# emilemathieu/RiemannHamiltonianMonteCarlo

Measured on AMD Instinct MI355X. Metric: leapfrog-steps/sec (whole node), higher is better.
Workload: dtype f64 (the two O(M D^2) contractions as exact int8-sliced integer GEMMs)

## Files before the change

### riemannhamiltonianmontecarlo_amd/csrc/metric_i8.hip.h

```cpp
#pragma once
#include <hip/hip_runtime.h>
#include <stdint.h>
#include <utility>
#include "plan.h"

typedef int i4v __attribute__((ext_vector_type(4)));
typedef int i16v __attribute__((ext_vector_type(16)));

#define I8_ROWB 32
__device__ __forceinline__ int i8_lds_off(int row, int half) { return row * I8_ROWB + ((half ^ ((row >> 3) & 1)) << 4); }

#ifndef I8_GC
#define I8_GC 4
#define I8_GP 8
#endif
#ifndef I8_DSPREAD
#define I8_DSPREAD 1
#endif
__device__ __forceinline__ bool i8_tile_of_block(int b, int nCB, int nPB, int& cb, int& pb) {
  if (nCB < 8) {
    if (b >= nCB * nPB) return false;
    cb = b % nCB;
    pb = b / nCB;
    return true;
// ... 41 lines not shown
}
#ifndef I8_ASMFRAG
#define I8_ASMFRAG 1
#endif

#ifndef I8_ABLATE
#define I8_ABLATE 0
#endif
template <int S, class F>
__device__ __forceinline__ double i8_combine(F&& acc_of) {
  double val = 0.0;
#pragma unroll
  for (int g = S - 1; g >= 0; --g) val = val * 0.00390625 + (double)acc_of(g);
  return val;
}

#ifndef I8_NBUF4
#define I8_NBUF4 1
#endif
template <int S, int WN, int TN>
constexpr int i8_nbuf() {
  constexpr int ROWS = I8_BM + 32 * TN * WN, NT = 128 * WN, NU = (2 * ROWS + NT - 1) / NT;
  return (I8_NBUF4 && S <= 4 && 2 * ROWS == NU * NT && 4 * S * ROWS * 32 <= 140 * 1024) ? 4 : 3;
}

template <int S, int WN, int TN, int PIN, bool RAW = false, class Epilogue>
__device__ __forceinline__ void gemm_i8_tile(const int8_t* __restrict__ Vs, const int8_t* __restrict__ Zs, int nCp, int NPp, int nks_total, int nks,
                                             int cb, int pb, int rows_real, int cols_real, Epilogue&& epi) {
  constexpr int BM = I8_BM, BN = 32 * TN * WN, ROWS = BM + BN, NT = 128 * WN;
  constexpr int STAGE = S * ROWS * I8_ROWB;
  constexpr int NU = (2 * ROWS + NT - 1) / NT;
  static_assert((2 * ROWS) % 64 == 0, "whole waves of 16-byte units");
  extern __shared__ __attribute__((aligned(16))) unsigned char lds[];
  const int t = threadIdx.x, lane = t & 63, wave = t >> 6;
  const int wm = wave & 1, wn = wave >> 1;
  const size_t strideV = (size_t)nks_total * nCp * 32, strideZ = (size_t)nks_total * NPp * 32;
  const int8_t* gbase[NU];
  size_t gstep[NU], gslice[NU];
  unsigned goff[NU];
  int lbase[NU];
  bool on[NU];
  int n_on = 0;
#pragma unroll
  for (int k = 0; k < NU; ++k) {
    const int u = t + k * NT;
    on[k] = (u & ~63) < 2 * ROWS;
// ... 120 lines not shown
        for (int a = 0; a < 2; ++a) fa[(i + 1) & 1][a] = *(const i4v*)(bc + (i + 1) * ROWS * I8_ROWB + fragA + a * 32 * I8_ROWB);
      }
      if (spread && (ALLON || ks + PD < nks)) gl1(kpre, wr, i);
      if (PIN) __builtin_amdgcn_sched_barrier(0);
#pragma unroll
      for (int j = S - 1 - i; j >= 0; --j) {
#pragma unroll
        for (int a = 0; a < 2; ++a)
#pragma unroll
          for (int b = 0; b < TN; ++b)
            acc[i + j][a][b] = __builtin_amdgcn_mfma_i32_32x32x32_i8(fa[i & 1][a], fb[j][b], acc[i + j][a][b], 0, 0, 0);
        if (PIN && i == 0) __builtin_amdgcn_sched_barrier(0);
      }
      if (PIN) __builtin_amdgcn_sched_barrier(0);
    }
    }
    }
    if constexpr (NBUF == 3) { if (ALLON || ks + 2 < nks) retire_older(); else wait_vmcnt<0>(); }
    else wait_vmcnt<(PD - 1) * S * NU>();
    if (!(I8_ABLATE & 4)) __builtin_amdgcn_s_barrier();
    cur = nxt;
  }
  if (ALLON) wait_vmcnt<0>();
#pragma unroll
  for (int a = 0; a < 2; ++a)
#pragma unroll
    for (int b = 0; b < TN; ++b)
#pragma unroll
      for (int r = 0; r < 16; ++r) {
        const int row = cb * BM + wm * 64 + a * 32 + (r & 3) + 8 * (r >> 2) + 4 * (lane >> 5);
        const int col = pb * BN + wn * 32 * TN + b * 32 + (lane & 31);
        if constexpr (RAW) {
#pragma unroll
          for (int g = 0; g < S; ++g) epi(row, col, g, acc[g][a][b][r]);
        } else {
          epi(row, col, i8_combine<S>([&](int g) { return acc[g][a][b][r]; }));
        }
      }
}

template <int S, int WN, int TN>
constexpr int i8_lds_bytes() { return i8_nbuf<S, WN, TN>() * S * (I8_BM + 32 * TN * WN) * I8_ROWB; }

template <int S, int WN, int TN, int PIN>
__global__ __launch_bounds__(128 * WN) __attribute__((amdgpu_waves_per_eu(WN >= 2 ? WN / 2 : 1, WN >= 4 ? WN / 2 : 2))) void k_gemm_i8_probe(const int8_t* __restrict__ Vs, const int8_t* __restrict__ Zs, int nCp, int NPp, int nks,
                                                            int nC, int NP, double* __restrict__ C) {
  int cb, pb;
  if (!i8_tile_of_block(blockIdx.x, nCp / I8_BM, NPp / (32 * TN * WN), cb, pb)) return;
  gemm_i8_tile<S, WN, TN, PIN>(Vs, Zs, nCp, NPp, nks, nks, cb, pb, nC - cb * I8_BM, NP - pb * 32 * TN * WN,
                          [&](int row, int col, double val) {
#ifdef I8_PROBE_NOSTORE
                            if (val == 1.2345e300)
#endif
                            C[(size_t)row * NPp + col] = val; });
}

template <int S>
__device__ __forceinline__ void split_digits(long long N, int (&d)[S]) {
#pragma unroll
  for (int k = 0; k < S; ++k) {
    const int b = (int)(signed char)(N & 0xFF);
    d[k] = b;
    N = (N - b) >> 8;
  }
}

struct I8Pairs {
  const short* pa;
  const short* pb;
  const double* scale;
  int NP, NPp;
  const int* cexp;
};

__global__ __launch_bounds__(256) void k_zmax(const double* __restrict__ Xt, int M, int Mp, I8Pairs pr, int* __restrict__ ze,
                                              double* __restrict__ scale) {
  __shared__ double red[256];
// ... 150 lines not shown

struct I8Delta {
  const unsigned long long* dsel;
  const int* rebase;
  double cscale;
  int need_lo, need_hi;
  const double* Gbase;
  unsigned long long* count = nullptr;
  __device__ __forceinline__ bool skip() const;
};
__device__ __forceinline__ int i8_delta_slices(unsigned long long bits) {
  const double mx = __longlong_as_double((long long)bits);
  if (mx <= 0.49 * 4294967296.0) return 4;
  if (mx <= 0.49 * 1099511627776.0) return 5;
  return 6;
}

__device__ __forceinline__ bool I8Delta::skip() const {
  if (!dsel) return false;
  const int need = i8_delta_slices(*dsel);
  return need < need_lo || need > need_hi;
}

template <int S, int WN, int TN>
__device__ __forceinline__ void assemble_i8_body(const int8_t* __restrict__ Vs, const int8_t* __restrict__ Zs, int nCp, int nks_total,
                                                 int ks0, int nk, int accumulate, const I8Pairs& pr, int n_chains, const int* __restrict__ phase,
                                                 const int* __restrict__ vbad, int DP, double inv_alpha, double* __restrict__ Gq,
                                                 size_t plane_stride, const int* __restrict__ vexp, int npb, const I8Delta& dl) {
  int cb, pb;
  if (!i8_tile_of_block(blockIdx.x, nCp / I8_BM, npb, cb, pb)) return;
  const int per = (nk + (int)gridDim.y - 1) / (int)gridDim.y;
  const int kb = ks0 + (int)blockIdx.y * per, kn = min(per, ks0 + nk - kb);
  double* __restrict__ Gout = Gq + (size_t)blockIdx.y * plane_stride;
  const bool first = blockIdx.y == 0;
  constexpr int BN = 32 * TN * WN;
  __shared__ double s_cmul[I8_BM];
  __shared__ double s_pscale[BN];
  __shared__ int s_coff[I8_BM];
  __shared__ int s_poff[BN];
  for (int i = threadIdx.x; i < I8_BM + BN; i += 128 * WN) {
    if (i < I8_BM) {
      const int c = cb * I8_BM + i;
      const bool ok = c < n_chains && phase[min(c, n_chains - 1)] == 1;
      s_coff[i] = ok ? ((dl.rebase && dl.rebase[c]) ? 3 : 1) : 0;
      s_cmul[i] = ok ? (vbad[c] ? __builtin_nan("") : ldexp(dl.cscale, -vexp[c])) : 0.0;
    } else {
      const int j = i - I8_BM, p = pb * BN + j;
      const bool ok = p < pr.NP;
      const int a = ok ? pr.pa[p] : 0, b = ok ? pr.pb[p] : 0;
      s_poff[j] = ok ? a * DP + b : -1;
      s_pscale[j] = ok ? (a == b ? -pr.scale[p] : pr.scale[p]) : 0.0;
    }
  }
  __syncthreads();
  gemm_i8_tile<S, WN, TN, (WN == 4)>(Vs + (size_t)kb * nCp * 32, Zs + (size_t)kb * pr.NPp * 32, nCp, pr.NPp, nks_total, kn, cb, pb,
                                     n_chains - cb * I8_BM, pr.NP - pb * 32 * TN * WN, [&](int c, int p, double val) {
    const int ci = c - cb * I8_BM, pj = p - pb * BN;
    const int off = s_poff[pj];
    const double ps = s_pscale[pj];
    const bool ok = s_coff[ci] != 0 && off >= 0;
    double* gp = Gout + (size_t)min(c, n_chains - 1) * DP * DP + max(off, 0);
    double g = (val * fabs(ps)) * s_cmul[ci];
    if (accumulate & 1) g += *gp;
    else if ((accumulate & 2) && s_coff[ci] != 3) g += dl.Gbase ? dl.Gbase[(size_t)min(c, n_chains - 1) * DP * DP + max(off, 0)] : *gp;
    else if (ps < 0.0 && first) g += inv_alpha;
    if (ok) *gp = g;
  });
}
template <int S, int WN, int TN>
__global__ __launch_bounds__(128 * WN) __attribute__((amdgpu_waves_per_eu(WN / 2, WN / 2))) void k_assemble_i8(const int8_t* __restrict__ Vs, const int8_t* __restrict__ Zs, int nCp, int nks_total,
                                                          int ks0, int nk, int accumulate, I8Pairs pr, int n_chains, const int* __restrict__ phase,
                                                          const int* __restrict__ vbad, int DP, double inv_alpha, double* __restrict__ Gq,
                                                          size_t plane_stride, const int* __restrict__ vexp, int npb, I8Delta dl) {
  if (dl.skip()) return;
  assemble_i8_body<S, WN, TN>(Vs, Zs, nCp, nks_total, ks0, nk, accumulate, pr, n_chains, phase, vbad, DP, inv_alpha, Gq, plane_stride, vexp, npb, dl);
}
__device__ __forceinline__ int i8_delta_pick(const I8Delta& dl, int seff) {
  const int need = i8_delta_slices(*dl.dsel);
  return seff == 6 ? need : (need == 6 ? 5 : 4);
}
__device__ __forceinline__ void i8_delta_count(const I8Delta& dl, int seff, int Sp) {
  if (dl.count && blockIdx.x == 0 && blockIdx.y == 0 && threadIdx.x == 0) atomicAdd(dl.count + 3 * (6 - seff) + (Sp - 4), 1ull);
}
template <int WN, int TN>
__global__ __launch_bounds__(128 * WN) __attribute__((amdgpu_waves_per_eu(WN / 2, WN / 2))) void k_assemble_i8_sel(const int8_t* __restrict__ Vs, size_t vplane, int seff, const int8_t* __restrict__ Zs, int nCp, int nks_total,
                                                          int ks0, int nk, int accumulate, I8Pairs pr, int n_chains, const int* __restrict__ phase,
                                                          const int* __restrict__ vbad, int DP, double inv_alpha, double* __restrict__ Gq,
                                                          size_t plane_stride, const int* __restrict__ vexp, int npb, I8Delta dl) {
  const int Sp = i8_delta_pick(dl, seff);
  i8_delta_count(dl, seff, Sp);
  dl.cscale = __builtin_ldexp(1.0, -8 * (seff - Sp));
  Vs += (size_t)(seff - Sp) * vplane;
  if (Sp == 6) assemble_i8_body<6, WN, TN>(Vs, Zs, nCp, nks_total, ks0, nk, accumulate, pr, n_chains, phase, vbad, DP, inv_alpha, Gq, plane_stride, vexp, npb, dl);
  else if (Sp == 5) assemble_i8_body<5, WN, TN>(Vs, Zs, nCp, nks_total, ks0, nk, accumulate, pr, n_chains, phase, vbad, DP, inv_alpha, Gq, plane_stride, vexp, npb, dl);
  else assemble_i8_body<4, WN, TN>(Vs, Zs, nCp, nks_total, ks0, nk, accumulate, pr, n_chains, phase, vbad, DP, inv_alpha, Gq, plane_stride, vexp, npb, dl);
}

template <int S>
__device__ __forceinline__ void assemble_i8_tail_body(
    const int8_t* __restrict__ Vs, const int8_t* __restrict__ Zs, int nCp, int NPp, int NP, int nks_total, int ks0, int nk, int n_chains, int pb32_0,
    int ntail, int* __restrict__ Tq) {
  const int nCB = nCp / I8_BM;
  const int cb = blockIdx.x % nCB, tb = blockIdx.x / nCB;
  const int per = (nk + (int)gridDim.y - 1) / (int)gridDim.y;
  const int kb = ks0 + (int)blockIdx.y * per, kn = min(per, ks0 + nk - kb);
  int* __restrict__ T = Tq + (size_t)blockIdx.y * S * nCp * 32 * ntail;
  const int pb32 = pb32_0 + tb;
  if (kn <= 0) {
    for (int i = threadIdx.x; i < S * I8_BM * 32; i += 128) {
      const int g = i / (I8_BM * 32), r = i % (I8_BM * 32);
      T[((size_t)g * nCp + cb * I8_BM + (r >> 5)) * 32 * ntail + tb * 32 + (r & 31)] = 0;
    }
    return;
  }
  gemm_i8_tile<S, 1, 1, 0, true>(Vs + (size_t)kb * nCp * 32, Zs + (size_t)kb * NPp * 32, nCp, NPp, nks_total, kn, cb, pb32, n_chains - cb * I8_BM,
                                 NP - pb32 * 32, [&](int c, int p, int g, int a) {
    T[((size_t)g * nCp + c) * 32 * ntail + (p - pb32_0 * 32)] = a;
  });
// ... 160 lines not shown
#pragma unroll
    for (int s = 0; s < S; ++s) w[s] = 0;
#pragma unroll
    for (int k = 0; k < 4; ++k) {
      int d[S];
      split_digits<S>((long long)rint(ldexp(ok ? q[k] : 0.0, shf)), d);
#pragma unroll
      for (int s = 0; s < S; ++s) w[s] |= (d[S - 1 - s] & 0xFF) << (8 * k);
    }
    const int kp = q4 >> 3, k4 = q4 & 7;
#pragma unroll
    for (int s = 0; s < S; ++s) *(int*)(Qs + (((size_t)s * nkp + kp) * nCp + c) * 32 + 4 * k4) = w[s];
  };
#pragma unroll
  for (int i = 0; i < QMAX; ++i)
    if (t + 256 * i < nq) put(t + 256 * i, qv[i]);
  for (int q4 = t + 256 * QMAX; q4 < nq; q4 += 256) {
    double mag;
    const double q[4] = {entry(4 * q4, mag), entry(4 * q4 + 1, mag), entry(4 * q4 + 2, mag), entry(4 * q4 + 3, mag)};
    put(q4, q);
  }
}

template <int S, int WN, int TN>
__global__ __launch_bounds__(128 * WN) __attribute__((amdgpu_waves_per_eu(WN / 2, WN / 2))) void k_leverage_i8(
    const int8_t* __restrict__ Qs, const int8_t* __restrict__ Zt, int nCp, int NRp, int nkp_total, int kp0, int nk, int accumulate, int mulc,
    int n_chains, int Mp, const int* __restrict__ phase, const double* __restrict__ qscale, const double* __restrict__ zscale,
    const double* __restrict__ crow, double* __restrict__ R, size_t plane_stride) {
  int cb, rb;
  if (!i8_tile_of_block(blockIdx.x, nCp / I8_BM, NRp / (32 * TN * WN), cb, rb)) return;
  const int per = (nk + (int)gridDim.y - 1) / (int)gridDim.y;
  const int kb = kp0 + (int)blockIdx.y * per, kn = min(per, kp0 + nk - kb);
  double* __restrict__ Rout = R + (size_t)blockIdx.y * plane_stride;
  constexpr int BN = 32 * TN * WN;
  __shared__ double s_q[I8_BM], s_z[BN];
  __shared__ int s_ok[I8_BM];
  for (int i = threadIdx.x; i < I8_BM + BN; i += 128 * WN) {
    if (i < I8_BM) {
      const int c = cb * I8_BM + i;
      const bool ok = c < n_chains && phase[min(c, n_chains - 1)] == 1;
      s_ok[i] = ok ? 1 : 0;
      s_q[i] = ok ? qscale[c] : 0.0;
    } else {
      const int n = rb * BN + (i - I8_BM);
      s_z[i - I8_BM] = n < NRp ? zscale[n] : 0.0;
    }
  }
  __syncthreads();
  gemm_i8_tile<S, WN, TN, (WN == 4)>(Qs + (size_t)kb * nCp * 32, Zt + (size_t)kb * NRp * 32, nCp, NRp, nkp_total, kn, cb, rb,
                                     n_chains - cb * I8_BM, Mp - rb * 32 * TN * WN, [&](int c, int n, double val) {
    const int ci = c - cb * I8_BM;
    const bool ok = s_ok[ci] != 0 && n < Mp;
    const size_t o = (size_t)min(c, n_chains - 1) * Mp + min(n, Mp - 1);
    double r = val * s_q[ci] * s_z[n - rb * BN];
    if (mulc) r *= crow[o];
    if (accumulate) r += Rout[o];
    if (ok) Rout[o] = r;
  });
}
```

### riemannhamiltonianmontecarlo_amd/csrc/plan.h

```cpp
#pragma once
#include "../../include/rmhmc.h"

#include <stddef.h>
#include <stdint.h>
#include <string.h>

#include <algorithm>

#define RM_LD 66

#define FS_D 8
#define FS_WAVES 4
#define FS_PT 104

#define MS_MAXMP 2048
#define MS_GLD 34

template <int NB>
constexpr int ms_lds_doubles(int Mp) {
  return 64 * RM_LD + 32 * MS_GLD + 4 * (16 * NB) * (16 * NB) + 2 * Mp + 12 * 32 + 4 * 40;
}

#define I8_BM 128
constexpr int i8_tile_wn(int S) { return S <= 6 ? 4 : 2; }
constexpr int i8_tile_tn(int) { return 1; }

#define AMH_MAX_ONCHIP_ROWS (256 * 48)

struct Options {
  int64_t graph = 1, sorted = 1, inflight = 32, cdyn = 1, crestore = 1, i8_force_rebase = 0;
  int64_t ccache = 1, medium = 1, fused = 1, hmc_traj_maxn = -1, fsplit = 0, nsplit_max = 64, nsplit_waves = -1, i8_tail = -1,
          i8_delta = 1, i8_delta_inner = 1;
};
struct OptionDesc { const char* key; int64_t Options::*slot; bool create_only; int64_t lo, hi; };
inline const OptionDesc kOptions[] = {
    {"graph", &Options::graph, false, 0, 1},
    {"sorted", &Options::sorted, false, 0, 1},
    {"inflight", &Options::inflight, false, 0, 1 << 20},
    {"cdyn", &Options::cdyn, false, 0, 1},
    {"crestore", &Options::crestore, false, 0, 1},
    {"i8_force_rebase", &Options::i8_force_rebase, false, 0, 1},
    {"ccache", &Options::ccache, true, 0, 1},
    {"medium", &Options::medium, true, 0, 1},
    {"fused", &Options::fused, true, 0, 1},
    {"hmc_traj_maxn", &Options::hmc_traj_maxn, true, -1, (int64_t)1 << 40},
    {"fsplit", &Options::fsplit, true, 0, 64},
    {"nsplit_max", &Options::nsplit_max, true, 1, 1 << 20},
    {"nsplit_waves", &Options::nsplit_waves, true, -1, 1 << 20},
    {"i8_tail", &Options::i8_tail, true, -1, 1},
    {"i8_delta", &Options::i8_delta, true, 0, 1},
    {"i8_delta_inner", &Options::i8_delta_inner, true, 0, 1},
};
inline const OptionDesc* find_option(const char* key) {
  if (!key) return nullptr;
  for (const OptionDesc& d : kOptions)
    if (!strcmp(d.key, key)) return &d;
  return nullptr;
}
enum OptionError { OPT_OK, OPT_UNKNOWN, OPT_CREATE_ONLY, OPT_RANGE };
inline OptionError check_option(const OptionDesc* d, int64_t value, bool at_create) {
  if (!d) return OPT_UNKNOWN;
  if (d->create_only && !at_create) return OPT_CREATE_ONLY;
  if (value < d->lo || value > d->hi) return OPT_RANGE;
  return OPT_OK;
}

struct PlanCheck { int code; const char* msg; };
inline PlanCheck plan_check(int64_t M, int32_t D, int64_t n_chains, int32_t dtype, uint32_t flags) {
  auto no = [](int code, const char* m) { return PlanCheck{code, m}; };
  if (M <= 0 || D <= 0 || n_chains <= 0) return no(RMHMC_ERR_INVALID, "rmhmc_create: bad shape");
  if (dtype != RMHMC_F64) return no(RMHMC_ERR_UNSUPPORTED, "rmhmc_create: only float64 is built (the reference is float64)");
  if (D > 256) return no(RMHMC_ERR_UNSUPPORTED, "rmhmc_create: D > 256 is not supported (64 < D <= 256 uses the blocked large-D path)");
  if (flags & RMHMC_FLAG_ORACLE_LITERAL) return no(RMHMC_ERR_UNSUPPORTED, "rmhmc_create: the literal variant exists only in the CPU oracle");
  if (M > (int64_t)1 << 30 || n_chains > (int64_t)1 << 30) return no(RMHMC_ERR_UNSUPPORTED, "rmhmc_create: M or n_chains too large");
// ... 138 lines not shown
```

### riemannhamiltonianmontecarlo_amd/csrc/rmhmc_hip.hip

```cpp
#include "../../include/rmhmc.h"
#include "../../include/rmhmc_amh.h"
#include "../../include/rmhmc_iwls.h"
#include "../../include/rmhmc_gibbs.h"
#include "plan.h"
#include "kernels.hip.h"
#include "fused_small.hip.h"
#include "large_d.hip.h"
#include "metric_i8.hip.h"
#include "medium_step.hip.h"
#include "amh.hip.h"
#include "iwls.hip.h"
#include "gibbs.hip.h"

#include <algorithm>
#include <chrono>
#include <cmath>
#include <cstdio>
#include <cstdlib>
#include <cstring>
#include <map>
#include <string>
#include <vector>

namespace {
// ... 202 lines not shown
  });
}

template <int S, int WN, int TN>
void launch_assemble_i8_t(rmhmc_ctx* ctx, Group& g, const double* v, hipStream_t st, int part, bool delta = false, int seff = 6, int need_lo = 0,
                          int need_hi = 0) {
  const size_t vplane = (size_t)ctx->i8_nks * g.nCp * 32;
  const int8_t* const Vs = g.Vs + (delta ? (size_t)(seff - S) * vplane : 0);
  const I8Delta dl{delta ? g.dmax : nullptr, delta ? g.rebase : nullptr, delta ? std::ldexp(1.0, -8 * (seff - S)) : 1.0, need_lo, need_hi,
                   (delta && ctx->big) ? g.Gbase : nullptr};
  const int* const vexp = delta ? g.vexp_d : g.vexp;
  const int acc0 = delta ? 2 : 0;
  if (part == 0) {
    if (delta) {
      (void)hipMemsetAsync(g.dmax, 0, sizeof(unsigned long long), st);
      hipLaunchKernelGGL((k_vsplit<S, true>), dim3((unsigned)((g.n + 7) / 8)), dim3(256), 0, st, v, ctx->Mp, g.n, g.ch.phase, ctx->i8_nks, g.nCp, g.Vs,
                         g.vbad, ctx->D, ctx->DP, ctx->dd.inv_alpha, g.ch.Gq, g.vexp, VDelta{g.vexp_d, g.rebase, g.dmax, (int)ctx->opt.i8_force_rebase});
      return;
    }
    hipLaunchKernelGGL((k_vsplit<S>), dim3((unsigned)((g.n + 7) / 8)), dim3(256), 0, st, v, ctx->Mp, g.n, g.ch.phase, ctx->i8_nks, g.nCp, g.Vs, g.vbad,
                       ctx->D, ctx->DP, ctx->dd.inv_alpha, g.ch.Gq, g.vexp, VDelta{});
    return;
  }
  constexpr int lds = i8_lds_bytes<S, WN, TN>();
  const I8Geometry t = i8_geometry(*ctx, g.nCp, WN, TN, WN == 4);
  if (ctx->ksplit_a > 1) {
    const size_t plane = (size_t)g.n * ctx->DP * ctx->DP;
    hipLaunchKernelGGL((k_assemble_i8<S, WN, TN>), dim3(t.nblk_main, (unsigned)ctx->ksplit_a), dim3(128 * WN), lds, st, g.Vs, ctx->d_Zs, g.nCp, ctx->i8_nks,
                       0, ctx->i8_nks, 0, ctx->pairs, g.n, g.ch.phase, g.vbad, ctx->DP, ctx->dd.inv_alpha, g.Gpart, plane, g.vexp, t.npb,
                       I8Delta{nullptr, nullptr, 1.0, 0, 0, nullptr});
    hipLaunchKernelGGL(k_sum_planes, dim3((unsigned)((plane + 255) / 256)), dim3(256), 0, st, g.ch.Gq, g.Gpart, ctx->ksplit_a, plane, plane);
    return;
  }
  for (int ks0 = 0; ks0 < ctx->i8_nks; ks0 += ctx->i8_chunk) {
    const int nk = std::min(ctx->i8_chunk, ctx->i8_nks - ks0);
    if (t.nblk_main)
      hipLaunchKernelGGL((k_assemble_i8<S, WN, TN>), dim3(t.nblk_main), dim3(128 * WN), lds, st, Vs, ctx->d_Zs, g.nCp,
                         ctx->i8_nks, ks0, nk, (ks0 > 0 ? 1 : 0) | acc0, ctx->pairs, g.n, g.ch.phase, g.vbad, ctx->DP, ctx->dd.inv_alpha, g.ch.Gq, (size_t)0, vexp, t.npb, dl);
    if (t.tail) {
      const int pieces = i8_tail_pieces(*ctx, t, nk);
      hipLaunchKernelGGL((k_assemble_i8_tail<S>), dim3((unsigned)(t.nCB * t.ntail), (unsigned)pieces), dim3(128), (i8_lds_bytes<S, 1, 1>()), st, Vs, ctx->d_Zs,
                         g.nCp, ctx->pairs.NPp, ctx->pairs.NP, ctx->i8_nks, ks0, nk, g.n, t.pb32_0, t.ntail, g.Tq, dl);
      hipLaunchKernelGGL((k_assemble_i8_tailsum<S>), dim3((unsigned)(((size_t)g.n * 32 * t.ntail + 255) / 256)), dim3(256), 0, st, g.Tq, pieces, g.nCp, t.ntail,
                         t.pb32_0, (ks0 > 0 ? 1 : 0) | acc0, ctx->pairs, g.n, g.ch.phase, g.vbad, ctx->DP, ctx->dd.inv_alpha, g.ch.Gq, vexp, dl);
    }
  }
}
void launch_assemble_i8_delta(rmhmc_ctx* ctx, Group& g, hipStream_t st, int seff) {
  constexpr int WN = 4, TN = 1;
  const size_t vplane = (size_t)ctx->i8_nks * g.nCp * 32;
  const I8Delta dl{g.dmax, g.rebase, 1.0, 0, 0, ctx->big ? g.Gbase : nullptr};
  const I8Geometry t = i8_geometry(*ctx, g.nCp, WN, TN);
  constexpr int lds = i8_lds_bytes<6, WN, TN>() > i8_lds_bytes<4, WN, TN>() ? i8_lds_bytes<6, WN, TN>() : i8_lds_bytes<4, WN, TN>();
  static_assert(lds >= (i8_lds_bytes<5, WN, TN>()), "dynamic LDS of the widest instantiation");
  constexpr int lds_t = i8_lds_bytes<6, 1, 1>() > i8_lds_bytes<4, 1, 1>() ? i8_lds_bytes<6, 1, 1>() : i8_lds_bytes<4, 1, 1>();
  static_assert(lds_t >= (i8_lds_bytes<5, 1, 1>()), "dynamic LDS of the widest tail instantiation");
  I8Delta dlc = dl;
  dlc.count = g.dcount;
  for (int ks0 = 0; ks0 < ctx->i8_nks; ks0 += ctx->i8_chunk) {
    const int nk = std::min(ctx->i8_chunk, ctx->i8_nks - ks0);
    if (t.nblk_main)
      hipLaunchKernelGGL((k_assemble_i8_sel<WN, TN>), dim3(t.nblk_main), dim3(128 * WN), lds, st, g.Vs, vplane, seff, ctx->d_Zs, g.nCp, ctx->i8_nks, ks0, nk,
                         (ks0 > 0 ? 1 : 0) | 2, ctx->pairs, g.n, g.ch.phase, g.vbad, ctx->DP, ctx->dd.inv_alpha, g.ch.Gq, (size_t)0, g.vexp_d, t.npb,
                         ks0 == 0 ? dlc : dl);
    if (t.tail) {
      const int pieces = i8_tail_pieces(*ctx, t, nk);
      hipLaunchKernelGGL(k_assemble_i8_tail_sel, dim3((unsigned)(t.nCB * t.ntail), (unsigned)pieces), dim3(128), lds_t, st, g.Vs, vplane, seff, ctx->d_Zs,
                         g.nCp, ctx->pairs.NPp, ctx->pairs.NP, ctx->i8_nks, ks0, nk, g.n, t.pb32_0, t.ntail, g.Tq, (ks0 == 0 && !t.nblk_main) ? dlc : dl);
      hipLaunchKernelGGL(k_assemble_i8_tailsum_sel, dim3((unsigned)(((size_t)g.n * 32 * t.ntail + 255) / 256)), dim3(256), 0, st, seff, g.Tq, pieces, g.nCp, t.ntail,
                         t.pb32_0, (ks0 > 0 ? 1 : 0) | 2, ctx->pairs, g.n, g.ch.phase, g.vbad, ctx->DP, ctx->dd.inv_alpha, g.ch.Gq, g.vexp_d, dl);
    }
  }
}
template <int S, int WN, int TN>
void launch_leverage_i8_t(rmhmc_ctx* ctx, Group& g, hipStream_t st, int part) {
  if (part == 0) {
    hipLaunchKernelGGL((k_qsplit<S>), dim3((unsigned)g.n), dim3(256), 0, st, g.ch.trj.Ginv, ctx->DP, ctx->pairs, g.ch.phase, ctx->i8_nkp, g.nCp,
                       g.Qs, g.qscale);
    return;
  }
  const int nCB = g.nCp / I8_BM, nRB = ctx->i8_NRp / (32 * TN * WN);
  constexpr int lds = i8_lds_bytes<S, WN, TN>();
  const unsigned nblk = (unsigned)(nCB < 8 ? nCB * nRB : (nCB + 7) / 8 * 8 * nRB);
  if (ctx->ksplit_l > 1) {
    const size_t plane = (size_t)g.n * ctx->Mp;
    hipLaunchKernelGGL((k_leverage_i8<S, WN, TN>), dim3(nblk, (unsigned)ctx->ksplit_l), dim3(128 * WN), lds, st, g.Qs, ctx->d_Zt, g.nCp, ctx->i8_NRp,
                       ctx->i8_nkp, 0, ctx->i8_nkp, 0, (ctx->big || g.ctile) ? 0 : 1, g.n, ctx->Mp, g.ch.phase, g.qscale, ctx->d_zscale, g.ch.rv2, g.Rpart, plane);
    hipLaunchKernelGGL(k_sum_planes, dim3((unsigned)((plane + 255) / 256)), dim3(256), 0, st, g.ch.rv0, g.Rpart, ctx->ksplit_l, plane, plane);
    return;
  }
  for (int kp0 = 0; kp0 < ctx->i8_nkp; kp0 += ctx->i8_chunk) {
    const int nk = std::min(ctx->i8_chunk, ctx->i8_nkp - kp0);
    hipLaunchKernelGGL((k_leverage_i8<S, WN, TN>), dim3(nblk), dim3(128 * WN), lds, st, g.Qs, ctx->d_Zt, g.nCp,
                       ctx->i8_NRp, ctx->i8_nkp, kp0, nk, kp0 > 0 ? 1 : 0, (ctx->big || g.ctile) ? 0 : 1, g.n, ctx->Mp, g.ch.phase, g.qscale, ctx->d_zscale,
                       g.ch.rv2, g.ch.rv0, (size_t)0);
  }
}
void launch_assemble(rmhmc_ctx* ctx, Group& g, const double* v, bool inner = false, bool delta = false, bool keep_base = false) {
  if (ctx->i8 && delta && ctx->big)
    launch(ctx, "vsplit", [&](hipStream_t st) { launch_assemble_i8_t<6, 4, 1>(ctx, g, v, st, 0, true); });
  if (ctx->i8 && delta && inner) {
    launch(ctx, "assemble_i8_inner_delta", [&](hipStream_t st) { launch_assemble_i8_delta(ctx, g, st, 5); });
    return;
  }
  if (ctx->i8 && delta) {
    launch(ctx, "assemble_i8_delta", [&](hipStream_t st) { launch_assemble_i8_delta(ctx, g, st, 6); });
    return;
  }
  if (ctx->i8) {
    if (ctx->big)
      launch(ctx, "vsplit", [&](hipStream_t st) { I8_SWITCH(ctx, (launch_assemble_i8_t<S_, WN_, TN_>(ctx, g, v, st, 0))); });
    const int suse = (inner && ctx->i8_inner_drop && ctx->i8S == 6) ? 5 : ctx->i8S;
    launch(ctx, suse == ctx->i8S ? "assemble_i8" : "assemble_i8_inner", [&](hipStream_t st) {
      I8_SWITCH_S(suse, (launch_assemble_i8_t<S_, WN_, TN_>(ctx, g, v, st, 1)));
      if (keep_base && ctx->big && g.Gbase)
        (void)hipMemcpyAsync(g.Gbase, g.ch.Gq, sizeof(double) * (size_t)g.n * ctx->DP * ctx->DP, hipMemcpyDeviceToDevice, st);
    });
    return;
// ... 458 lines not shown
      RC(sync(ctx));
      int* d_cexp;
      RC(dalloc(ctx, &d_cexp, DP));
      RC(dalloc(ctx, &ctx->d_cmin, DP)); RC(dalloc(ctx, &ctx->d_cmax, DP));
      ctx->pairs = I8Pairs{d_pa, d_pb, d_scale, ctx->NP, ctx->NPp, d_cexp};
      RC(dalloc(ctx, &ctx->d_Zs, S * nks * NPp * 32));
      RC(dalloc(ctx, &ctx->d_Zt, S * nkp * NRp * 32));
      RC(dalloc(ctx, &ctx->d_zre, NRp)); RC(dalloc(ctx, &ctx->d_zscale, NRp));
      RC(dalloc(ctx, &g.Vs, S * nks * nCp * 32));
      RC(dalloc(ctx, &g.vbad, nCp));
      RC(dalloc(ctx, &g.vexp, nCp));
      RC(dalloc(ctx, &g.vexp_d, nCp)); RC(dalloc(ctx, &g.rebase, nCp)); RC(dalloc(ctx, &g.dmax, (size_t)1));
      RC(dalloc(ctx, &g.dcount, (size_t)6));
      if (!ctx->big) { ch.i8_vbad = g.vbad; ch.i8_dmax = g.dmax; }
      if (ctx->gbase) RC(dalloc(ctx, &g.Gbase, n * DP * DP));
      RC(dalloc(ctx, &g.Qs, S * nkp * nCp * 32));
      RC(dalloc(ctx, &g.qscale, nCp));
      if (ctx->tail_acc) RC(dalloc(ctx, &g.Tq, (size_t)ctx->tail_pieces * S * nCp * 32 * ctx->tail_blocks));
      if (ctx->ksplit_l > 1) RC(dalloc(ctx, &g.Rpart, (size_t)ctx->ksplit_l * n * Mp));
      for (int sv = ctx->i8S == 6 ? 4 : ctx->i8S; sv <= ctx->i8S; ++sv)
        I8_SWITCH_S(sv, {
          constexpr int lds = i8_lds_bytes<S_, WN_, TN_>();
          RC(raise_lds(ctx, k_assemble_i8<S_, WN_, TN_>, lds));
          RC(raise_lds(ctx, k_leverage_i8<S_, WN_, TN_>, lds));
          RC(raise_lds(ctx, k_assemble_i8_tail<S_>, (i8_lds_bytes<S_, 1, 1>())));
        });
      if (ctx->i8S == 6) {
        RC(raise_lds(ctx, k_assemble_i8_sel<4, 1>, std::max((i8_lds_bytes<6, 4, 1>()), (i8_lds_bytes<4, 4, 1>()))));
        RC(raise_lds(ctx, k_assemble_i8_tail_sel, std::max((i8_lds_bytes<6, 1, 1>()), (i8_lds_bytes<4, 1, 1>()))));
      }
    }
    if (ctx->gpart_planes) RC(dalloc(ctx, &g.Gpart, (size_t)ctx->gpart_planes * n * DP * DP));
    RC(dalloc(ctx, &ctx->d_z, n * (size_t)D)); RC(dalloc(ctx, &ctx->d_ulen, n)); RC(dalloc(ctx, &ctx->d_gdir, n)); RC(dalloc(ctx, &ctx->d_uacc, n));
    if (ctx->big) RC(dalloc(ctx, &ctx->d_Wd, n * (size_t)ctx->nbk * 4096));
    if (ctx->hpart_at_create) RC(dalloc(ctx, &ctx->d_hpart, (size_t)ctx->npairs * n * Mp));
    fill_int(ctx, ch.cstale, 1, n);
    RC(dalloc(ctx, &ctx->d_nsteps, n)); RC(dalloc(ctx, &ctx->d_dir, n)); RC(dalloc(ctx, &ctx->d_done, 1)); RC(dalloc(ctx, &ctx->d_steps0, n));
    RC(dalloc(ctx, &ctx->d_miniter, 1));
    RC(dalloc(ctx, &ctx->d_orig, n)); RC(dalloc(ctx, &ctx->d_T, 2 * n));
    if (ctx->medium) RC(ctx->NB == 1 ? (raise_lds_medium<1, 0, 1, 2, 3, 4>(ctx)) : (raise_lds_medium<2, 0, 1, 2>(ctx)));
    if (ctx->fused) RC(raise_lds(ctx, k_fused_small, MAX_LDS));
    RC(sync(ctx));
    return RMHMC_OK;
  };
  rc = body();
  if (rc != RMHMC_OK) {
    snprintf(g_err, 512, "%s", ctx->err);
    rmhmc_destroy(ctx);
    return rc;
  }
  apply_runtime_options(ctx);
// ... 1294 lines not shown
```

Baseline: 558,500.

## Load Z operand directly into registers for S=4 int8 GEMM tiles

```diff
diff --git a/riemannhamiltonianmontecarlo_amd/csrc/metric_i8.hip.h b/riemannhamiltonianmontecarlo_amd/csrc/metric_i8.hip.h
--- a/riemannhamiltonianmontecarlo_amd/csrc/metric_i8.hip.h
+++ b/riemannhamiltonianmontecarlo_amd/csrc/metric_i8.hip.h
@@ -87,6 +87,25 @@
 constexpr int i8_nbuf() {
   constexpr int ROWS = I8_BM + 32 * TN * WN, NT = 128 * WN, NU = (2 * ROWS + NT - 1) / NT;
   return (I8_NBUF4 && S <= 4 && 2 * ROWS == NU * NT && 4 * S * ROWS * 32 <= 140 * 1024) ? 4 : 3;
+}
+
+template <int S, int TN, int BN, bool RAW, class Epilogue>
+__device__ __forceinline__ void i8_tile_epilogue(const i16v (&acc)[S][2][TN], int cb, int pb, int wm, int wn, int lane, Epilogue&& epi) {
+#pragma unroll
+  for (int a = 0; a < 2; ++a)
+#pragma unroll
+    for (int b = 0; b < TN; ++b)
+#pragma unroll
+      for (int r = 0; r < 16; ++r) {
+        const int row = cb * I8_BM + wm * 64 + a * 32 + (r & 3) + 8 * (r >> 2) + 4 * (lane >> 5);
+        const int col = pb * BN + wn * 32 * TN + b * 32 + (lane & 31);
+        if constexpr (RAW) {
+#pragma unroll
+          for (int g = 0; g < S; ++g) epi(row, col, g, acc[g][a][b][r]);
+        } else {
+          epi(row, col, i8_combine<S>([&](int g) { return acc[g][a][b][r]; }));
+        }
+      }
 }
 
 template <int S, int WN, int TN, int PIN, bool RAW = false, class Epilogue>
@@ -253,37 +272,154 @@
     cur = nxt;
   }
   if (ALLON) wait_vmcnt<0>();
-#pragma unroll
-  for (int a = 0; a < 2; ++a)
-#pragma unroll
-    for (int b = 0; b < TN; ++b)
-#pragma unroll
-      for (int r = 0; r < 16; ++r) {
-        const int row = cb * BM + wm * 64 + a * 32 + (r & 3) + 8 * (r >> 2) + 4 * (lane >> 5);
-        const int col = pb * BN + wn * 32 * TN + b * 32 + (lane & 31);
-        if constexpr (RAW) {
-#pragma unroll
-          for (int g = 0; g < S; ++g) epi(row, col, g, acc[g][a][b][r]);
-        } else {
-          epi(row, col, i8_combine<S>([&](int g) { return acc[g][a][b][r]; }));
-        }
+  i8_tile_epilogue<S, TN, BN, RAW>(acc, cb, pb, wm, wn, lane, epi);
+}
+
+
+#ifndef I8_ZRING
+#define I8_ZRING 3
+#endif
+constexpr bool i8_zdirect_tile(int S, int WN, int TN) { return S == 4 && WN == 4 && TN == 1; }
+template <int S, int P>
+constexpr int i8_zd_lds_bytes() { return (P + 1) * S * I8_BM * I8_ROWB; }
+
+__device__ __forceinline__ void gbl_load_b128(i4v& r, unsigned off, const void* base) {
+  asm volatile("global_load_dwordx4 %0, %1, %2" : "+v"(r) : "v"(off), "s"(base) : "memory");
+}
+template <int N>
+__device__ __forceinline__ void wait_vmcnt(i4v& a, i4v& b, i4v& c, i4v& d) {
+  static_assert(N >= 0 && N < 64, "vmcnt immediate");
+  asm volatile("s_waitcnt vmcnt(%4)" : "+v"(a), "+v"(b), "+v"(c), "+v"(d) : "n"(N) : "memory");
+}
+
+template <int S, int P, class Epilogue>
+__device__ __forceinline__ void gemm_i8_tile_zd(const int8_t* __restrict__ Vs, const int8_t* __restrict__ Zs, int nCp, int NPp, int nks_total, int nks,
+                                                int cb, int pb, int rows_real, int cols_real, Epilogue&& epi) {
+  constexpr int BM = I8_BM, BN = 128, NBUF = P + 1;
+  constexpr int SLICE = BM * I8_ROWB, STAGE = S * SLICE;
+  constexpr int ND = S / 2, Q = S + ND;
+  static_assert(S == 4, "four fb registers per ring slot are named on the waits");
+  static_assert(P >= 2 && (P - 1) * Q < 64, "vmcnt immediate");
+  extern __shared__ __attribute__((aligned(16))) unsigned char lds[];
+  const int t = threadIdx.x, lane = t & 63, wave = __builtin_amdgcn_readfirstlane(t >> 6);
+  const int wm = wave & 1, wn = wave >> 1;
+  const size_t strideV = (size_t)nks_total * nCp * 32, strideZ = (size_t)nks_total * NPp * 32;
+  const size_t stepV = (size_t)nCp * 32, stepZ = (size_t)NPp * 32;
+  const int sp = wave >> 2, u = t & 255, urow = u >> 1;
+  const int8_t* const va = Vs + ((size_t)cb * BM) * 32 + sp * strideV;
+  const unsigned goff = (unsigned)(urow * 32 + (((u & 1) ^ ((urow >> 3) & 1)) << 4));
+  const int lbase = sp * SLICE + (wave & 3) * 64 * 16;
+  auto dma = [&](int ks, int buf, int q) {
+    __builtin_amdgcn_global_load_lds((gbl_ptr_t)(va + (2 * q * strideV + (size_t)ks * stepV) + goff),
+                                     (lds_ptr_t)(lds + buf * STAGE + 2 * q * SLICE + lbase), 16, 0, 0);
+  };
+  const int8_t* const zw = Zs + ((size_t)pb * BN + wn * 32) * 32;
+  const unsigned zoff = (unsigned)((lane & 31) * 32 + (lane >> 5) * 16);
+  auto zld = [&](i4v& r, int ks, int j) { gbl_load_b128(r, zoff, zw + (j * strideZ + (size_t)ks * stepZ)); };
+
+  i16v acc[S][2][1];
+#pragma unroll
+  for (int g = 0; g < S; ++g)
+#pragma unroll
+    for (int a = 0; a < 2; ++a)
+#pragma unroll
+      for (int r = 0; r < 16; ++r) acc[g][a][0][r] = 0;
+  const bool work = wm * 64 < rows_real && wn * 32 < cols_real;
+  if (!work) {
+#pragma unroll
+    for (int d = 0; d < P; ++d)
+#pragma unroll
+      for (int q = 0; q < ND; ++q) dma(min(d, nks - 1), d, q);
+    wait_vmcnt<(P - 1) * ND>();
+    __builtin_amdgcn_s_barrier();
+    int wr = NBUF - 1;
+    for (int ks = 0; ks < nks; ++ks) {
+#pragma unroll
+      for (int q = 0; q < ND; ++q) dma(min(ks + P, nks - 1), wr, q);
+      wait_vmcnt<(P - 1) * ND>();
+      __builtin_amdgcn_s_barrier();
+      wr = wr + 1 >= NBUF ? 0 : wr + 1;
+    }
+    wait_vmcnt<0>();
+  } else {
+    i4v fb[P][S], fa[2][2];
+#pragma unroll
+    for (int d = 0; d < P; ++d)
+#pragma unroll
+      for (int j = 0; j < S; ++j) fb[d][j] = i4v{0, 0, 0, 0};
+#pragma unroll
+    for (int d = 0; d < P; ++d) {
+      const int kd = min(d, nks - 1);
+#pragma unroll
+      for (int i = 0; i < S; ++i) {
+        if (i < ND) dma(kd, d, i);
+        zld(fb[d][S - 1 - i], kd, S - 1 - i);
       }
-}
-
-template <int S, int WN, int TN>
-constexpr int i8_lds_bytes() { return i8_nbuf<S, WN, TN>() * S * (I8_BM + 32 * TN * WN) * I8_ROWB; }
-
-template <int S, int WN, int TN, int PIN>
+    }
+    wait_vmcnt<(P - 1) * Q>(fb[0][0], fb[0][1], fb[0][2], fb[0][3]);
+    __builtin_amdgcn_s_barrier();
+    const int fragA = i8_lds_off(wm * 64 + (lane & 31), lane >> 5);
+    const unsigned a0 = (unsigned)(size_t)(lds_ptr_t)(lds) + fragA;
+    int cur = 0;
+    auto stage = [&]<int R>(std::integral_constant<int, R>, int ks) {
+      const int wr = cur == 0 ? NBUF - 1 : cur - 1;
+      const int kpre = min(ks + P, nks - 1);
+      const unsigned aA = a0 + cur * STAGE;
+      fa[0][0] = lds_read_b128<0>(aA);
+      fa[0][1] = lds_read_b128<32 * I8_ROWB>(aA);
+      [&]<int... I>(std::integer_sequence<int, I...>) {
+        ([&] {
+          constexpr int i = I;
+          if constexpr (i + 1 < S) {
+            fa[(i + 1) & 1][0] = lds_read_b128<(i + 1) * SLICE>(aA);
+            fa[(i + 1) & 1][1] = lds_read_b128<(i + 1) * SLICE + 32 * I8_ROWB>(aA);
+          }
+          if constexpr (i < ND) dma(kpre, wr, i);
+          wait_lgkm<(i + 1 < S) ? 2 : 0>(fa[i & 1][0], fa[i & 1][1]);
+#pragma unroll
+          for (int j = S - 1 - i; j >= 0; --j) {
+            acc[i + j][0][0] = __builtin_amdgcn_mfma_i32_32x32x32_i8(fa[i & 1][0], fb[R][j], acc[i + j][0][0], 0, 0, 0);
+            acc[i + j][1][0] = __builtin_amdgcn_mfma_i32_32x32x32_i8(fa[i & 1][1], fb[R][j], acc[i + j][1][0], 0, 0, 0);
+          }
+          __builtin_amdgcn_sched_barrier(0);
+          zld(fb[R][S - 1 - i], kpre, S - 1 - i);
+        }(), ...);
+      }(std::make_integer_sequence<int, S>{});
+      constexpr int R1 = (R + 1) % P;
+      wait_vmcnt<(P - 1) * Q>(fb[R1][0], fb[R1][1], fb[R1][2], fb[R1][3]);
+      __builtin_amdgcn_s_barrier();
+      cur = cur + 1 >= NBUF ? 0 : cur + 1;
+    };
+    for (int ks = 0; ks < nks; ks += P) {
+      bool more = true;
+      [&]<int... R>(std::integer_sequence<int, R...>) {
+        ((more = more && ks + R < nks, more ? stage(std::integral_constant<int, R>{}, ks + R) : (void)0), ...);
+      }(std::make_integer_sequence<int, P>{});
+    }
+#pragma unroll
+    for (int d = 0; d < P; ++d) wait_vmcnt<0>(fb[d][0], fb[d][1], fb[d][2], fb[d][3]);
+  }
+  i8_tile_epilogue<S, 1, BN, false>(acc, cb, pb, wm, wn, lane, epi);
+}
+
+template <int S, int WN, int TN, bool ZD = false>
+constexpr int i8_lds_bytes() {
+  if (ZD && i8_zdirect_tile(S, WN, TN)) return i8_zd_lds_bytes<S, I8_ZRING>();
+  return i8_nbuf<S, WN, TN>() * S * (I8_BM + 32 * TN * WN) * I8_ROWB;
+}
+
+template <int S, int WN, int TN, int PIN, int ZP = 0>
 __global__ __launch_bounds__(128 * WN) __attribute__((amdgpu_waves_per_eu(WN >= 2 ? WN / 2 : 1, WN >= 4 ? WN / 2 : 2))) void k_gemm_i8_probe(const int8_t* __restrict__ Vs, const int8_t* __restrict__ Zs, int nCp, int NPp, int nks,
                                                             int nC, int NP, double* __restrict__ C) {
   int cb, pb;
   if (!i8_tile_of_block(blockIdx.x, nCp / I8_BM, NPp / (32 * TN * WN), cb, pb)) return;
-  gemm_i8_tile<S, WN, TN, PIN>(Vs, Zs, nCp, NPp, nks, nks, cb, pb, nC - cb * I8_BM, NP - pb * 32 * TN * WN,
-                          [&](int row, int col, double val) {
+  auto epi = [&](int row, int col, double val) {
 #ifdef I8_PROBE_NOSTORE
-                            if (val == 1.2345e300)
+    if (val == 1.2345e300)
 #endif
-                            C[(size_t)row * NPp + col] = val; });
+    C[(size_t)row * NPp + col] = val; };
+  if constexpr (ZP > 0) gemm_i8_tile_zd<S, ZP>(Vs, Zs, nCp, NPp, nks, nks, cb, pb, nC - cb * I8_BM, NP - pb * 32 * TN * WN, epi);
+  else gemm_i8_tile<S, WN, TN, PIN>(Vs, Zs, nCp, NPp, nks, nks, cb, pb, nC - cb * I8_BM, NP - pb * 32 * TN * WN, epi);
 }
 
 template <int S>
@@ -480,7 +616,7 @@
   return need < need_lo || need > need_hi;
 }
 
-template <int S, int WN, int TN>
+template <int S, int WN, int TN, bool ZD = false>
 __device__ __forceinline__ void assemble_i8_body(const int8_t* __restrict__ Vs, const int8_t* __restrict__ Zs, int nCp, int nks_total,
                                                  int ks0, int nk, int accumulate, const I8Pairs& pr, int n_chains, const int* __restrict__ phase,
                                                  const int* __restrict__ vbad, int DP, double inv_alpha, double* __restrict__ Gq,
@@ -511,8 +647,7 @@
     }
   }
   __syncthreads();
-  gemm_i8_tile<S, WN, TN, (WN == 4)>(Vs + (size_t)kb * nCp * 32, Zs + (size_t)kb * pr.NPp * 32, nCp, pr.NPp, nks_total, kn, cb, pb,
-                                     n_chains - cb * I8_BM, pr.NP - pb * 32 * TN * WN, [&](int c, int p, double val) {
+  auto epi = [&](int c, int p, double val) {
     const int ci = c - cb * I8_BM, pj = p - pb * BN;
     const int off = s_poff[pj];
     const double ps = s_pscale[pj];
@@ -523,15 +658,21 @@
     else if ((accumulate & 2) && s_coff[ci] != 3) g += dl.Gbase ? dl.Gbase[(size_t)min(c, n_chains - 1) * DP * DP + max(off, 0)] : *gp;
     else if (ps < 0.0 && first) g += inv_alpha;
     if (ok) *gp = g;
-  });
-}
-template <int S, int WN, int TN>
+  };
+  if constexpr (ZD && i8_zdirect_tile(S, WN, TN))
+    gemm_i8_tile_zd<S, I8_ZRING>(Vs + (size_t)kb * nCp * 32, Zs + (size_t)kb * pr.NPp * 32, nCp, pr.NPp, nks_total, kn, cb, pb, n_chains - cb * I8_BM,
+                                 pr.NP - pb * 32 * TN * WN, epi);
+  else
+    gemm_i8_tile<S, WN, TN, (WN == 4)>(Vs + (size_t)kb * nCp * 32, Zs + (size_t)kb * pr.NPp * 32, nCp, pr.NPp, nks_total, kn, cb, pb,
+                                       n_chains - cb * I8_BM, pr.NP - pb * 32 * TN * WN, epi);
+}
+template <int S, int WN, int TN, bool ZD = false>
 __global__ __launch_bounds__(128 * WN) __attribute__((amdgpu_waves_per_eu(WN / 2, WN / 2))) void k_assemble_i8(const int8_t* __restrict__ Vs, const int8_t* __restrict__ Zs, int nCp, int nks_total,
                                                           int ks0, int nk, int accumulate, I8Pairs pr, int n_chains, const int* __restrict__ phase,
                                                           const int* __restrict__ vbad, int DP, double inv_alpha, double* __restrict__ Gq,
                                                           size_t plane_stride, const int* __restrict__ vexp, int npb, I8Delta dl) {
   if (dl.skip()) return;
-  assemble_i8_body<S, WN, TN>(Vs, Zs, nCp, nks_total, ks0, nk, accumulate, pr, n_chains, phase, vbad, DP, inv_alpha, Gq, plane_stride, vexp, npb, dl);
+  assemble_i8_body<S, WN, TN, ZD>(Vs, Zs, nCp, nks_total, ks0, nk, accumulate, pr, n_chains, phase, vbad, DP, inv_alpha, Gq, plane_stride, vexp, npb, dl);
 }
 __device__ __forceinline__ int i8_delta_pick(const I8Delta& dl, int seff) {
   const int need = i8_delta_slices(*dl.dsel);
@@ -540,7 +681,7 @@
 __device__ __forceinline__ void i8_delta_count(const I8Delta& dl, int seff, int Sp) {
   if (dl.count && blockIdx.x == 0 && blockIdx.y == 0 && threadIdx.x == 0) atomicAdd(dl.count + 3 * (6 - seff) + (Sp - 4), 1ull);
 }
-template <int WN, int TN>
+template <int WN, int TN, bool ZD = false>
 __global__ __launch_bounds__(128 * WN) __attribute__((amdgpu_waves_per_eu(WN / 2, WN / 2))) void k_assemble_i8_sel(const int8_t* __restrict__ Vs, size_t vplane, int seff, const int8_t* __restrict__ Zs, int nCp, int nks_total,
                                                           int ks0, int nk, int accumulate, I8Pairs pr, int n_chains, const int* __restrict__ phase,
                                                           const int* __restrict__ vbad, int DP, double inv_alpha, double* __restrict__ Gq,
@@ -551,7 +692,7 @@
   Vs += (size_t)(seff - Sp) * vplane;
   if (Sp == 6) assemble_i8_body<6, WN, TN>(Vs, Zs, nCp, nks_total, ks0, nk, accumulate, pr, n_chains, phase, vbad, DP, inv_alpha, Gq, plane_stride, vexp, npb, dl);
   else if (Sp == 5) assemble_i8_body<5, WN, TN>(Vs, Zs, nCp, nks_total, ks0, nk, accumulate, pr, n_chains, phase, vbad, DP, inv_alpha, Gq, plane_stride, vexp, npb, dl);
-  else assemble_i8_body<4, WN, TN>(Vs, Zs, nCp, nks_total, ks0, nk, accumulate, pr, n_chains, phase, vbad, DP, inv_alpha, Gq, plane_stride, vexp, npb, dl);
+  else assemble_i8_body<4, WN, TN, ZD>(Vs, Zs, nCp, nks_total, ks0, nk, accumulate, pr, n_chains, phase, vbad, DP, inv_alpha, Gq, plane_stride, vexp, npb, dl);
 }
 
 template <int S>
@@ -758,7 +899,7 @@
   }
 }
 
-template <int S, int WN, int TN>
+template <int S, int WN, int TN, bool ZD = false>
 __global__ __launch_bounds__(128 * WN) __attribute__((amdgpu_waves_per_eu(WN / 2, WN / 2))) void k_leverage_i8(
     const int8_t* __restrict__ Qs, const int8_t* __restrict__ Zt, int nCp, int NRp, int nkp_total, int kp0, int nk, int accumulate, int mulc,
     int n_chains, int Mp, const int* __restrict__ phase, const double* __restrict__ qscale, const double* __restrict__ zscale,
@@ -783,8 +924,7 @@
     }
   }
   __syncthreads();
-  gemm_i8_tile<S, WN, TN, (WN == 4)>(Qs + (size_t)kb * nCp * 32, Zt + (size_t)kb * NRp * 32, nCp, NRp, nkp_total, kn, cb, rb,
-                                     n_chains - cb * I8_BM, Mp - rb * 32 * TN * WN, [&](int c, int n, double val) {
+  auto epi = [&](int c, int n, double val) {
     const int ci = c - cb * I8_BM;
     const bool ok = s_ok[ci] != 0 && n < Mp;
     const size_t o = (size_t)min(c, n_chains - 1) * Mp + min(n, Mp - 1);
@@ -792,5 +932,11 @@
     if (mulc) r *= crow[o];
     if (accumulate) r += Rout[o];
     if (ok) Rout[o] = r;
-  });
-}
+  };
+  if constexpr (ZD && i8_zdirect_tile(S, WN, TN))
+    gemm_i8_tile_zd<S, I8_ZRING>(Qs + (size_t)kb * nCp * 32, Zt + (size_t)kb * NRp * 32, nCp, NRp, nkp_total, kn, cb, rb, n_chains - cb * I8_BM,
+                                 Mp - rb * 32 * TN * WN, epi);
+  else
+    gemm_i8_tile<S, WN, TN, (WN == 4)>(Qs + (size_t)kb * nCp * 32, Zt + (size_t)kb * NRp * 32, nCp, NRp, nkp_total, kn, cb, rb,
+                                       n_chains - cb * I8_BM, Mp - rb * 32 * TN * WN, epi);
+}
diff --git a/riemannhamiltonianmontecarlo_amd/csrc/plan.h b/riemannhamiltonianmontecarlo_amd/csrc/plan.h
--- a/riemannhamiltonianmontecarlo_amd/csrc/plan.h
+++ b/riemannhamiltonianmontecarlo_amd/csrc/plan.h
@@ -30,7 +30,7 @@
 struct Options {
   int64_t graph = 1, sorted = 1, inflight = 32, cdyn = 1, crestore = 1, i8_force_rebase = 0;
   int64_t ccache = 1, medium = 1, fused = 1, hmc_traj_maxn = -1, fsplit = 0, nsplit_max = 64, nsplit_waves = -1, i8_tail = -1,
-          i8_delta = 1, i8_delta_inner = 1;
+          i8_delta = 1, i8_delta_inner = 1, i8_zdirect = 1;
 };
 struct OptionDesc { const char* key; int64_t Options::*slot; bool create_only; int64_t lo, hi; };
 inline const OptionDesc kOptions[] = {
@@ -50,6 +50,7 @@
     {"i8_tail", &Options::i8_tail, true, -1, 1},
     {"i8_delta", &Options::i8_delta, true, 0, 1},
     {"i8_delta_inner", &Options::i8_delta_inner, true, 0, 1},
+    {"i8_zdirect", &Options::i8_zdirect, true, 0, 1},
 };
 inline const OptionDesc* find_option(const char* key) {
   if (!key) return nullptr;
diff --git a/riemannhamiltonianmontecarlo_amd/csrc/rmhmc_hip.hip b/riemannhamiltonianmontecarlo_amd/csrc/rmhmc_hip.hip
--- a/riemannhamiltonianmontecarlo_amd/csrc/rmhmc_hip.hip
+++ b/riemannhamiltonianmontecarlo_amd/csrc/rmhmc_hip.hip
@@ -248,21 +248,26 @@
                        ctx->D, ctx->DP, ctx->dd.inv_alpha, g.ch.Gq, g.vexp, VDelta{});
     return;
   }
-  constexpr int lds = i8_lds_bytes<S, WN, TN>();
   const I8Geometry t = i8_geometry(*ctx, g.nCp, WN, TN, WN == 4);
+  auto main_tiles = [&](dim3 grid, auto... args) {
+    if (i8_zdirect_tile(S, WN, TN) && ctx->opt.i8_zdirect)
+      hipLaunchKernelGGL((k_assemble_i8<S, WN, TN, true>), grid, dim3(128 * WN), (i8_lds_bytes<S, WN, TN, true>()), st, args...);
+    else
+      hipLaunchKernelGGL((k_assemble_i8<S, WN, TN>), grid, dim3(128 * WN), (i8_lds_bytes<S, WN, TN>()), st, args...);
+  };
   if (ctx->ksplit_a > 1) {
     const size_t plane = (size_t)g.n * ctx->DP * ctx->DP;
-    hipLaunchKernelGGL((k_assemble_i8<S, WN, TN>), dim3(t.nblk_main, (unsigned)ctx->ksplit_a), dim3(128 * WN), lds, st, g.Vs, ctx->d_Zs, g.nCp, ctx->i8_nks,
-                       0, ctx->i8_nks, 0, ctx->pairs, g.n, g.ch.phase, g.vbad, ctx->DP, ctx->dd.inv_alpha, g.Gpart, plane, g.vexp, t.npb,
-                       I8Delta{nullptr, nullptr, 1.0, 0, 0, nullptr});
+    main_tiles(dim3(t.nblk_main, (unsigned)ctx->ksplit_a), (const int8_t*)g.Vs, (const int8_t*)ctx->d_Zs, g.nCp, ctx->i8_nks,
+               0, ctx->i8_nks, 0, ctx->pairs, g.n, (const int*)g.ch.phase, (const int*)g.vbad, ctx->DP, ctx->dd.inv_alpha, g.Gpart, plane, (const int*)g.vexp, t.npb,
+               I8Delta{nullptr, nullptr, 1.0, 0, 0, nullptr});
     hipLaunchKernelGGL(k_sum_planes, dim3((unsigned)((plane + 255) / 256)), dim3(256), 0, st, g.ch.Gq, g.Gpart, ctx->ksplit_a, plane, plane);
     return;
   }
   for (int ks0 = 0; ks0 < ctx->i8_nks; ks0 += ctx->i8_chunk) {
     const int nk = std::min(ctx->i8_chunk, ctx->i8_nks - ks0);
     if (t.nblk_main)
-      hipLaunchKernelGGL((k_assemble_i8<S, WN, TN>), dim3(t.nblk_main), dim3(128 * WN), lds, st, Vs, ctx->d_Zs, g.nCp,
-                         ctx->i8_nks, ks0, nk, (ks0 > 0 ? 1 : 0) | acc0, ctx->pairs, g.n, g.ch.phase, g.vbad, ctx->DP, ctx->dd.inv_alpha, g.ch.Gq, (size_t)0, vexp, t.npb, dl);
+      main_tiles(dim3(t.nblk_main), Vs, (const int8_t*)ctx->d_Zs, g.nCp, ctx->i8_nks, ks0, nk, (ks0 > 0 ? 1 : 0) | acc0, ctx->pairs, g.n,
+                 (const int*)g.ch.phase, (const int*)g.vbad, ctx->DP, ctx->dd.inv_alpha, g.ch.Gq, (size_t)0, vexp, t.npb, dl);
     if (t.tail) {
       const int pieces = i8_tail_pieces(*ctx, t, nk);
       hipLaunchKernelGGL((k_assemble_i8_tail<S>), dim3((unsigned)(t.nCB * t.ntail), (unsigned)pieces), dim3(128), (i8_lds_bytes<S, 1, 1>()), st, Vs, ctx->d_Zs,
@@ -283,12 +288,16 @@
   static_assert(lds_t >= (i8_lds_bytes<5, 1, 1>()), "dynamic LDS of the widest tail instantiation");
   I8Delta dlc = dl;
   dlc.count = g.dcount;
+  auto main_tiles = [&](dim3 grid, auto... args) {
+    if (ctx->opt.i8_zdirect) hipLaunchKernelGGL((k_assemble_i8_sel<WN, TN, true>), grid, dim3(128 * WN), lds, st, args...);
+    else hipLaunchKernelGGL((k_assemble_i8_sel<WN, TN>), grid, dim3(128 * WN), lds, st, args...);
+  };
   for (int ks0 = 0; ks0 < ctx->i8_nks; ks0 += ctx->i8_chunk) {
     const int nk = std::min(ctx->i8_chunk, ctx->i8_nks - ks0);
     if (t.nblk_main)
-      hipLaunchKernelGGL((k_assemble_i8_sel<WN, TN>), dim3(t.nblk_main), dim3(128 * WN), lds, st, g.Vs, vplane, seff, ctx->d_Zs, g.nCp, ctx->i8_nks, ks0, nk,
-                         (ks0 > 0 ? 1 : 0) | 2, ctx->pairs, g.n, g.ch.phase, g.vbad, ctx->DP, ctx->dd.inv_alpha, g.ch.Gq, (size_t)0, g.vexp_d, t.npb,
-                         ks0 == 0 ? dlc : dl);
+      main_tiles(dim3(t.nblk_main), (const int8_t*)g.Vs, vplane, seff, (const int8_t*)ctx->d_Zs, g.nCp, ctx->i8_nks, ks0, nk, (ks0 > 0 ? 1 : 0) | 2, ctx->pairs,
+                 g.n, (const int*)g.ch.phase, (const int*)g.vbad, ctx->DP, ctx->dd.inv_alpha, g.ch.Gq, (size_t)0, (const int*)g.vexp_d, t.npb,
+                 ks0 == 0 ? dlc : dl);
     if (t.tail) {
       const int pieces = i8_tail_pieces(*ctx, t, nk);
       hipLaunchKernelGGL(k_assemble_i8_tail_sel, dim3((unsigned)(t.nCB * t.ntail), (unsigned)pieces), dim3(128), lds_t, st, g.Vs, vplane, seff, ctx->d_Zs,
@@ -306,20 +315,26 @@
     return;
   }
   const int nCB = g.nCp / I8_BM, nRB = ctx->i8_NRp / (32 * TN * WN);
-  constexpr int lds = i8_lds_bytes<S, WN, TN>();
   const unsigned nblk = (unsigned)(nCB < 8 ? nCB * nRB : (nCB + 7) / 8 * 8 * nRB);
+  auto tiles = [&](dim3 grid, auto... args) {
+    if (i8_zdirect_tile(S, WN, TN) && ctx->opt.i8_zdirect)
+      hipLaunchKernelGGL((k_leverage_i8<S, WN, TN, true>), grid, dim3(128 * WN), (i8_lds_bytes<S, WN, TN, true>()), st, args...);
+    else
+      hipLaunchKernelGGL((k_leverage_i8<S, WN, TN>), grid, dim3(128 * WN), (i8_lds_bytes<S, WN, TN>()), st, args...);
+  };
   if (ctx->ksplit_l > 1) {
     const size_t plane = (size_t)g.n * ctx->Mp;
-    hipLaunchKernelGGL((k_leverage_i8<S, WN, TN>), dim3(nblk, (unsigned)ctx->ksplit_l), dim3(128 * WN), lds, st, g.Qs, ctx->d_Zt, g.nCp, ctx->i8_NRp,
-                       ctx->i8_nkp, 0, ctx->i8_nkp, 0, (ctx->big || g.ctile) ? 0 : 1, g.n, ctx->Mp, g.ch.phase, g.qscale, ctx->d_zscale, g.ch.rv2, g.Rpart, plane);
+    tiles(dim3(nblk, (unsigned)ctx->ksplit_l), (const int8_t*)g.Qs, (const int8_t*)ctx->d_Zt, g.nCp, ctx->i8_NRp, ctx->i8_nkp, 0, ctx->i8_nkp, 0,
+          (ctx->big || g.ctile) ? 0 : 1, g.n, ctx->Mp, (const int*)g.ch.phase, (const double*)g.qscale, (const double*)ctx->d_zscale,
+          (const double*)g.ch.rv2, g.Rpart, plane);
     hipLaunchKernelGGL(k_sum_planes, dim3((unsigned)((plane + 255) / 256)), dim3(256), 0, st, g.ch.rv0, g.Rpart, ctx->ksplit_l, plane, plane);
     return;
   }
   for (int kp0 = 0; kp0 < ctx->i8_nkp; kp0 += ctx->i8_chunk) {
     const int nk = std::min(ctx->i8_chunk, ctx->i8_nkp - kp0);
-    hipLaunchKernelGGL((k_leverage_i8<S, WN, TN>), dim3(nblk), dim3(128 * WN), lds, st, g.Qs, ctx->d_Zt, g.nCp,
-                       ctx->i8_NRp, ctx->i8_nkp, kp0, nk, kp0 > 0 ? 1 : 0, (ctx->big || g.ctile) ? 0 : 1, g.n, ctx->Mp, g.ch.phase, g.qscale, ctx->d_zscale,
-                       g.ch.rv2, g.ch.rv0, (size_t)0);
+    tiles(dim3(nblk), (const int8_t*)g.Qs, (const int8_t*)ctx->d_Zt, g.nCp, ctx->i8_NRp, ctx->i8_nkp, kp0, nk, kp0 > 0 ? 1 : 0,
+          (ctx->big || g.ctile) ? 0 : 1, g.n, ctx->Mp, (const int*)g.ch.phase, (const double*)g.qscale, (const double*)ctx->d_zscale,
+          (const double*)g.ch.rv2, g.ch.rv0, (size_t)0);
   }
 }
 void launch_assemble(rmhmc_ctx* ctx, Group& g, const double* v, bool inner = false, bool delta = false, bool keep_base = false) {
@@ -824,11 +839,16 @@
         I8_SWITCH_S(sv, {
           constexpr int lds = i8_lds_bytes<S_, WN_, TN_>();
           RC(raise_lds(ctx, k_assemble_i8<S_, WN_, TN_>, lds));
+          if constexpr (i8_zdirect_tile(S_, WN_, TN_)) {
+            RC(raise_lds(ctx, k_assemble_i8<S_, WN_, TN_, true>, (i8_lds_bytes<S_, WN_, TN_, true>())));
+            RC(raise_lds(ctx, k_leverage_i8<S_, WN_, TN_, true>, (i8_lds_bytes<S_, WN_, TN_, true>())));
+          }
           RC(raise_lds(ctx, k_leverage_i8<S_, WN_, TN_>, lds));
           RC(raise_lds(ctx, k_assemble_i8_tail<S_>, (i8_lds_bytes<S_, 1, 1>())));
         });
       if (ctx->i8S == 6) {
         RC(raise_lds(ctx, k_assemble_i8_sel<4, 1>, std::max((i8_lds_bytes<6, 4, 1>()), (i8_lds_bytes<4, 4, 1>()))));
+        RC(raise_lds(ctx, k_assemble_i8_sel<4, 1, true>, std::max((i8_lds_bytes<6, 4, 1>()), (i8_lds_bytes<4, 4, 1, true>()))));
         RC(raise_lds(ctx, k_assemble_i8_tail_sel, std::max((i8_lds_bytes<6, 1, 1>()), (i8_lds_bytes<4, 1, 1>()))));
       }
     }
```

After: 565,600, median of 6. 1.01x the previous value.
